# starlingonearth/MASt3R-SLAM-Quality-dualTSDF

Measured on AMD Instinct MI355X. Metric: SLAM frames/sec (infer+match+TSDF+GN) @512x384, higher is better.
Workload: dtype bf16

## Files before the change

include/mslam_hip.h:

```cpp
#ifndef MSLAM_HIP_H
#define MSLAM_HIP_H

#include <stddef.h>
#include <stdint.h>

#ifdef __cplusplus
extern "C" {
#endif

#define MSLAM_OK 0
#define MSLAM_EINVAL (-1)
#define MSLAM_EHIP (-2)
#define MSLAM_ENOMEM (-3)
#define MSLAM_ENODEV (-4)

const char* mslam_last_error(void);
int mslam_abi_version(void);
int mslam_device_check(void);


int mslam_iter_proj(const float* rays_img_with_grad, const float* pts_3d_norm,
                    const float* p_init, float* p_new, uint8_t* converged, int b, int h, int w,
                    int n, int max_iter, float lambda_init, float cost_thresh, void* stream);

// ... 15 lines not shown
int mslam_gauss_newton_rays(float* Twc, const float* Xs, const float* Cs, const int64_t* ii,
                            const int64_t* jj, const int64_t* idx_ii2jj, const uint8_t* valid_match,
                            const float* Q, int num_poses, int num_points, int num_edges,
                            float sigma_ray, float sigma_dist, float C_thresh, float Q_thresh,
                            int max_iter, float delta_thresh, float* dx, void* workspace,
                            size_t workspace_bytes, void* stream);

int mslam_gauss_newton_calib(float* Twc, const float* Xs, const float* Cs, const float* K,
                             const int64_t* ii, const int64_t* jj, const int64_t* idx_ii2jj,
                             const uint8_t* valid_match, const float* Q, int num_poses, int num_points,
                             int num_edges, int height, int width, int pixel_border, float z_eps,
                             float sigma_pixel, float sigma_depth, float C_thresh, float Q_thresh,
                             int max_iter, float delta_thresh, float* dx, void* workspace,
                             size_t workspace_bytes, void* stream);

int mslam_gauss_newton_points(float* Twc, const float* Xs, const float* Cs, const int64_t* ii,
                              const int64_t* jj, const int64_t* idx_ii2jj, const uint8_t* valid_match,
                              const float* Q, int num_poses, int num_points, int num_edges,
                              float sigma_point, float C_thresh, float Q_thresh, int max_iter,
                              float delta_thresh, float* dx, void* workspace, size_t workspace_bytes,
                              void* stream);

int mslam_gn_begin(const int64_t* ii, const int64_t* jj, int num_poses, int num_edges, int num_points,
                   void* workspace, size_t workspace_bytes, void* stream);
int mslam_gn_compact(const float* Xs, const float* Cs, const int64_t* idx_ii2jj, const uint8_t* valid_match,
                     const float* Q, int num_poses, int num_points, int num_edges, int edge_begin,
                     int edge_count, float C_thresh, float Q_thresh, void* workspace, size_t workspace_bytes,
                     void* stream);
int mslam_gn_compact_at(const float* Xs, const float* Cs, const int64_t* idx_ii2jj, const uint8_t* valid_match,
                        const float* Q, int num_poses, int num_points, int num_edges, int edge_begin, int edge_count,
                        int slot_begin, int range_count, float C_thresh, float Q_thresh, void* workspace,
                        size_t workspace_bytes, void* stream);
int mslam_gn_accumulate(int kind, const float* Twc, const float* K, int num_poses, int num_points,
                        int num_edges, int edge_begin, int edge_count, float sigma_a, float sigma_b,
                        int height, int width, int pixel_border, float z_eps, float* Hs, float* gs,
                        void* workspace, size_t workspace_bytes, void* stream);
int mslam_gn_solve_retract(const float* Hs, const float* gs, int num_poses, int num_edges,
                           int num_points, float* Twc, float* dx, float delta_thresh, void* workspace,
                           size_t workspace_bytes, void* stream);
int mslam_gn_status(int* status4, int num_poses, int num_edges, int num_points, void* workspace,
                    size_t workspace_bytes, void* stream);

int mslam_sim3_act(const float* T, const float* X, float* Y, int num_poses, long long pts_per_pose,
                   int broadcast_pose, void* stream);
int mslam_sim3_op(int op, const float* A, const float* B, float* out, int n, int bcast_a, int bcast_b,
                  void* stream);

size_t mslam_tsdf_table_bytes(uint64_t capacity);
int mslam_tsdf_table_init(void* table, size_t table_bytes, uint64_t capacity, void* stream);

size_t mslam_tsdf_integrate_workspace_bytes(int n_points, double voxel_size, double trunc, double step_scale);
int mslam_tsdf_integrate(void* table, uint64_t capacity, const float* points_world, const double* conf,
                         const float* cam_origin, int n_points, double voxel_size, double trunc,
                         double max_weight, double step_scale, int shard_id, int num_shards,
                         void* workspace, size_t workspace_bytes, void* stream);

int mslam_tsdf_rehash(void* old_table, uint64_t old_capacity, void* new_table, uint64_t new_capacity, void* stream);
int mslam_tsdf_header(void* table, uint64_t capacity, uint32_t* out8_host, void* stream);

int mslam_tsdf_dump(void* table, uint64_t capacity, int64_t* keys, double* tsdf, double* weight,
                    uint32_t max_out, void* stream);

int mslam_tsdf_query(void* table, uint64_t capacity, const float* points, int n, double voxel_size,
                     double min_weight, double* value, double* grad, uint8_t* status, void* stream);

int mslam_tsdf_pose_step(void* table, uint64_t capacity, const float* points, const float* conf, int n,
                         float* pose, int points_in_camera_frame, double voxel_size, double min_weight,
                         double lambda, double damping, int update_pose, double* H_out, double* b_out,
                         int* used_out, void* workspace, size_t workspace_bytes, void* stream);

int mslam_tsdf_lookup7(void* table, uint64_t capacity, const float* points, int n, const float* pose,
                       double voxel_size, double* out, void* stream);
int mslam_tsdf_query_lookup(const double* lookup, int n, double voxel_size, double min_weight, double* value,
                            double* grad, uint8_t* status, void* stream);
int mslam_tsdf_pose_step_lookup(const double* lookup, const float* points, const float* conf, int n, float* pose,
                                int points_in_camera_frame, double voxel_size, double min_weight, double lambda,
                                double damping, int update_pose, double* H_out, double* b_out, int* used_out,
                                void* workspace, size_t workspace_bytes, void* stream);

size_t mslam_tsdf_mesh_workspace_bytes(uint64_t capacity);
int mslam_tsdf_mesh_keys(void* table, uint64_t capacity, double min_weight, int64_t* sort_keys, void* stream);
int mslam_tsdf_mesh_count(void* table, uint64_t capacity, double min_weight, double level, const int64_t* sorted_keys,
                          const int64_t* order, int32_t* counts, void* workspace, size_t workspace_bytes, void* stream);
int mslam_tsdf_mesh_emit(void* table, uint64_t capacity, double voxel_size, double min_weight, double level,
                         const int64_t* sorted_keys, const int64_t* order, const int64_t* vbase, const int64_t* fbase,
                         void* workspace, size_t workspace_bytes, float* vertices, float* normals, int32_t* faces,
                         int64_t n_vertices, int64_t n_faces, void* stream);
int mslam_tsdf_load(void* table, uint64_t capacity, const int64_t* keys, const double* tsdf, const double* weight,
                    int n, void* stream);

size_t mslam_tsdf_render_workspace_bytes(uint64_t capacity);
int mslam_tsdf_render_blocks(void* table, uint64_t capacity, double min_weight, void* workspace, size_t workspace_bytes,
                             void* stream);
int mslam_tsdf_render(void* table, uint64_t capacity, const float* rays, int h, int w, const float* pose8,
                      double voxel_size, double min_weight, double level, double near, double far, double step, int skip,
                      const void* workspace, size_t workspace_bytes, float* range, float* normal, uint8_t* hit,
                      void* stream);

size_t mslam_tsdf_color_bytes(uint64_t capacity);
int mslam_tsdf_color_init(void* color, size_t color_bytes, uint64_t capacity, void* stream);
int mslam_tsdf_integrate_color(void* table, uint64_t capacity, void* color, const float* points_world,
                               const double* conf, const float* rgb, const float* cam_origin, int n_points,
                               double voxel_size, double trunc, double step_scale, void* stream);
int mslam_tsdf_color_rehash(void* old_table, uint64_t old_capacity, const void* old_color, void* new_table,
                            uint64_t new_capacity, void* new_color, void* stream);
int mslam_tsdf_color_dump(void* table, uint64_t capacity, const void* color, const int64_t* keys, int n, uint64_t* sums,
                          void* stream);
int mslam_tsdf_color_load(void* table, uint64_t capacity, void* color, const int64_t* keys, const uint64_t* sums, int n,
                          void* stream);
int mslam_tsdf_color_sample(void* table, uint64_t capacity, const void* color, const float* points, int n, int image_w,
                            double voxel_size, double default_r, double default_g, double default_b, float* out_rgb,
                            uint8_t* out_count, void* stream);

int mslam_mast3r_create(void** handle_out, const int* cfg9_host, void* const* weight_ptrs_host,
                        const long long* weight_numels_host, int n_weights, void* stream);
int mslam_mast3r_destroy(void* handle);
size_t mslam_mast3r_workspace_bytes(void* handle, int batch, int H, int W);

int mslam_mast3r_encode(void* handle, const float* img, int batch, int H, int W, float* feat_out,
                        void* workspace, size_t workspace_bytes, void* stream);

int mslam_mast3r_decode(void* handle, const float* feat1, const float* feat2, int batch, int H, int W,
                        float* X1, float* C1, float* D1, float* Q1, float* X2, float* C2, float* D2,
                        float* Q2, float* dec_last1, float* dec_last2, void* workspace,
                        size_t workspace_bytes, void* stream);

size_t mslam_track_workspace_bytes(int n_points);
int mslam_track_pose(int use_calib, float* T_rel, const float* Xf, const float* Xk, const int64_t* idx_f2k,
                     const float* Qk, const uint8_t* valid, int n_points, const float* K, int width,
                     int height, float sigma_a, float sigma_b, float huber, int pixel_border, float z_eps,
                     int first_iter, int max_iters, float rel_error, float delta_norm, void* status_out, void* workspace,
                     size_t workspace_bytes, void* stream);

size_t mslam_track_prepare_workspace_bytes(int n_points);
int mslam_track_prepare(const int64_t* idx_f2k, const uint8_t* valid_match, const float* Qff, const float* Qkf,
                        const float* Cf_sum, float inv_nf, const float* Ck_sum, float inv_nk, float C_conf, float Q_conf,
                        int n_points, const float* T_WCk, const float* T_WCf, float* Qk, float* Ck_avg,
                        uint8_t* valid_opt, uint8_t* valid_kf, float* T_rel, void* workspace, size_t workspace_bytes,
                        void* stream);
int mslam_track_verdict(const void* prepare_workspace, const void* status, int n_points, float* verdict6, void* stream);
int mslam_track_fuse(const float* T_WCk, const float* T_rel, const float* Xkf, const float* Ckf, const float* X_canon,
                     const float* C, int n_points, float* T_WCf, float* X_new, float* C_new, void* stream);

int mslam_gemm_bf16(const void* A, const void* W, const float* bias, const void* residual_f32, void* out,
                    int M, int N, int K, int act, int out_is_bf16, void* stream);
int mslam_gemm_tile_override(int M, int N, int K, int cfg);
int mslam_gemm_profile_begin(int M, int N, int K, int max_samples);
int mslam_gemm_profile_end(double* avg_us, double* min_us, int* samples);
int mslam_conv2d_nhwc_bf16(const void* in, const void* W, const float* bias, const void* residual_bf16,
                           void* out_bf16, int B, int H, int Wd, int Cin, int Cout, int ks, int stride,
                           int relu_in, int act, void* stream);
int mslam_attention_bf16(const void* Q, const void* K, const void* VT, void* O, int batch, int heads,
                         int nq, int nk, void* stream);
int mslam_layernorm_f32(const float* x, const float* w, const float* b, void* out_bf16, float* out_f32,
                        int rows, int D, float eps, void* stream);

size_t mslam_tsdf_local_workspace_bytes(int n_points);
int mslam_tsdf_local_build(const float* X_world, const float* C, const float* origin, const float* xyz_min,
                           const float* xyz_max, int n_points, int nx, int ny, int nz, double voxel_size,
                           double trunc, float min_confidence, float* tsdf, float* weights, void* workspace,
                           size_t workspace_bytes, void* stream);
int mslam_tsdf_local_raycast(const float* tsdf, int nx, int ny, int nz, const float* xyz_min,
                             const float* xyz_max, const float* X_original, const int64_t* sel_pix, int n_sel,
                             int n_samples, float max_displacement, float* surf, uint8_t* hit, void* stream);

int mslam_quality_reduce_grid(const float* x, const float* y, const uint8_t* valid, int h, int w, int ps, int mode,
                              double c_thr, double q_thr, float* out, void* stream);
int mslam_quality_classify(const float* delta_cov, const float* r, const float* u, int n, float thr_zr, float thr_zu,
                           float thr_dc, int64_t* cls, float* pri, void* stream);

int mslam_room_pair(const float* ki, const float* kj, int batch, int h, int w, int n_frames, double fx, double fy,
                    double cx, double cy, double noise, const double* Wm_3x24, const double* phase_24, float* X1,
                    float* C1, float* D1, float* Q1, float* X2, float* C2, float* D2, float* Q2, void* stream);

int mslam_remap_bilinear_u8(const uint8_t* src, int src_h, int src_w, int channels, const float* mapx,
                            const float* mapy, uint8_t* dst, int dst_h, int dst_w, void* stream);

int mslam_gemm_f64(const void* A, int a_is_f32, const void* B, int b_is_f32, int b_transposed, const double* centre,
                   const double* bias, double* out, int M, int N, int K, void* stream);

int mslam_asmk_aggregate(const float* des, const float* centroids, const int64_t* assign, const int64_t* uniq_words,
                         uint32_t* sig_out, int n_des, int m_assign, int dim, int n_uniq, int n_centroids, void* stream);
int mslam_asmk_search(const int32_t* entry_word, const uint32_t* entry_sig, const int32_t* img_start, int n_images,
                      const int32_t* q_words, const uint32_t* q_sig, int n_q, int sig_words, float similarity_threshold,
                      float alpha, double* scores, void* stream);

#ifdef __cplusplus
}
#endif
#endif
```

mast3r-slam-quality-dualtsdf_amd/csrc/attention.hip:

```cpp
#include <stdlib.h>
#include "common.h"
#include "gemm.h"

namespace mslam {

typedef __attribute__((ext_vector_type(8))) __bf16 bf16x8;
typedef __attribute__((ext_vector_type(4))) __bf16 bf16x4;
typedef __attribute__((ext_vector_type(16))) float f32x16;
typedef __attribute__((ext_vector_type(4))) unsigned int u32x4;

constexpr int KV_TILE = 64;
constexpr int AT_STAGE = 16384;
constexpr int OM_ROW = 68;
constexpr unsigned kAtOob = 0x80000000u;

#define MSLAM_LDS_PTR(p) ((__attribute__((address_space(3))) void*)(p))

template <int N>
__device__ __forceinline__ void at_wait_vmcnt() {
  __builtin_amdgcn_s_waitcnt((N & 15) | ((N >> 4) << 14) | 0x0F70);
}

template <int AT_SPLIT>
__global__ __launch_bounds__(128 * AT_SPLIT) void attention_kernel(const bf16* __restrict__ Q, const bf16* __restrict__ K,
                                                        const bf16* __restrict__ VT, bf16* __restrict__ O,
                                                        int heads, int nq, int nk) {
  extern __shared__ __attribute__((aligned(1024))) unsigned char smem[];
  const int t = threadIdx.x, lane = t & 63;
  const int wid = __builtin_amdgcn_readfirstlane(t >> 6);
  const int qg = wid & 1, sp = wid >> 1;
  const int h = lane >> 5, lq = lane & 31;
  const int head = blockIdx.y, b = blockIdx.z;
  const size_t bh = (size_t)b * heads + head;
  const int q_row = blockIdx.x * 64 + qg * 32 + lq;
  const bool q_ok = q_row < nq;

  bf16x8 qf[4];
#pragma unroll
  for (int s = 0; s < 4; s++) {
    const size_t qi = (bh * nq + (q_ok ? q_row : 0)) * 64 + 16 * s + 8 * h;
    qf[s] = __builtin_bit_cast(bf16x8, *reinterpret_cast<const u32x4*>(Q + qi));
  }

  const int ntiles = (nk + KV_TILE - 1) / KV_TILE;
  const int n_iter = (ntiles + AT_SPLIT - 1) / AT_SPLIT;
  const int t_begin = sp * n_iter;
  const int my_n = max(0, min(ntiles, t_begin + n_iter) - t_begin);

  const __amdgpu_buffer_rsrc_t rsK =
      __builtin_amdgcn_make_buffer_rsrc((void*)(K + bh * (size_t)nk * 64), 0, nk * 128, 0x00020000);
  const __amdgpu_buffer_rsrc_t rsV =
      __builtin_amdgcn_make_buffer_rsrc((void*)(VT + bh * 64 * (size_t)nk), 0, nk * 128, 0x00020000);
  const int chunk = (lane & 7) ^ (4 * qg + (lane >> 4));
  unsigned k_off[4], v_off[4];
#pragma unroll
  for (int i = 0; i < 4; i++) {
    const int row = (qg + 2 * i) * 8 + (lane >> 3);
    k_off[i] = (unsigned)(row * 64 + chunk * 8) * 2u;
    v_off[i] = (unsigned)(row * nk + chunk * 8) * 2u;
  }
  auto issue = [&](int stage, int tile) {
    unsigned char* base = smem + (sp * 2 + stage) * AT_STAGE + qg * 1024;
    const int kv0 = tile * KV_TILE;
    const unsigned v_bad = (unsigned)(nk - 1 - (kv0 + chunk * 8)) & kAtOob;
#pragma unroll
    for (int i = 0; i < 4; i++)
      __builtin_amdgcn_raw_ptr_buffer_load_lds(rsK, MSLAM_LDS_PTR(base + i * 2048), 16, k_off[i] + (unsigned)kv0 * 128u, 0, 0, 0);
#pragma unroll
    for (int i = 0; i < 4; i++)
      __builtin_amdgcn_raw_ptr_buffer_load_lds(rsV, MSLAM_LDS_PTR(base + 8192 + i * 2048), 16,
                                               (v_off[i] + (unsigned)kv0 * 2u) | v_bad, 0, 0, 0);
  };

  f32x16 o_acc[2];
#pragma unroll
  for (int dt = 0; dt < 2; dt++)
#pragma unroll
    for (int r = 0; r < 16; r++) o_acc[dt][r] = 0.0f;
  float m_run = -INFINITY, l_run = 0.0f;
  const float kLog2e = 1.4426950408889634f;
  const int kh = h ^ ((lq >> 1) & 7);

  auto compute = [&](int stage, int tile) {
    const unsigned char* sK = smem + (sp * 2 + stage) * AT_STAGE + lq * 128;
    const unsigned char* sV = sK + 8192;
    const int kv0 = tile * KV_TILE;
    f32x16 s_acc[2];
#pragma unroll
    for (int u = 0; u < 2; u++) {
#pragma unroll
      for (int r = 0; r < 16; r++) s_acc[u][r] = 0.0f;
#pragma unroll
      for (int s = 0; s < 4; s++) {
        const bf16x8 kf = *reinterpret_cast<const bf16x8*>(sK + u * 4096 + (((2 * s) ^ kh) * 16));
        s_acc[u] = __builtin_amdgcn_mfma_f32_32x32x16_bf16(kf, qf[s], s_acc[u], 0, 0, 0);
      }
    }
    if (kv0 + KV_TILE > nk) {
#pragma unroll
      for (int u = 0; u < 2; u++)
#pragma unroll
        for (int r = 0; r < 16; r++)
          if (kv0 + 32 * u + (r & 3) + 8 * (r >> 2) + 4 * h >= nk) s_acc[u][r] = -INFINITY;
    }
    float m_tile = -INFINITY;
#pragma unroll
    for (int u = 0; u < 2; u++)
#pragma unroll
      for (int r = 0; r < 16; r++) m_tile = fmaxf(m_tile, s_acc[u][r]);
    m_tile = fmaxf(m_tile, __shfl_xor(m_tile, 32, 64));
    const float m_new = fmaxf(m_run, m_tile);
    const float alpha = __builtin_amdgcn_exp2f((m_run - m_new) * kLog2e);
    const float neg_m = -m_new * kLog2e;
    float l_tile = 0.0f;
#pragma unroll
    for (int u = 0; u < 2; u++)
#pragma unroll
      for (int r = 0; r < 16; r++) {
        const float p = __builtin_amdgcn_exp2f(fmaf(s_acc[u][r], kLog2e, neg_m));
        s_acc[u][r] = p;
        l_tile += p;
      }
    l_tile += __shfl_xor(l_tile, 32, 64);
    l_run = l_run * alpha + l_tile;
    m_run = m_new;
#pragma unroll
    for (int dt = 0; dt < 2; dt++)
#pragma unroll
      for (int r = 0; r < 16; r++) o_acc[dt][r] *= alpha;
#pragma unroll
    for (int u = 0; u < 2; u++) {
#pragma unroll
      for (int s2 = 0; s2 < 2; s2++) {
        bf16x8 pf;
#pragma unroll
        for (int j = 0; j < 8; j++) pf[j] = (bf16)s_acc[u][8 * s2 + j];
        const int c0 = 4 * u + 2 * s2;
#pragma unroll
        for (int dt = 0; dt < 2; dt++) {
          const unsigned char* vrow = sV + dt * 4096 + 8 * h;
          const bf16x4 v0 = *reinterpret_cast<const bf16x4*>(vrow + ((c0 ^ ((lq >> 1) & 7)) * 16));
          const bf16x4 v1 = *reinterpret_cast<const bf16x4*>(vrow + (((c0 + 1) ^ ((lq >> 1) & 7)) * 16));
          bf16x8 vf;
          vf[0] = v0[0]; vf[1] = v0[1]; vf[2] = v0[2]; vf[3] = v0[3];
          vf[4] = v1[0]; vf[5] = v1[1]; vf[6] = v1[2]; vf[7] = v1[3];
          o_acc[dt] = __builtin_amdgcn_mfma_f32_32x32x16_bf16(vf, pf, o_acc[dt], 0, 0, 0);
        }
      }
    }
  };

  if (my_n > 0) issue(0, t_begin);
  if (my_n > 1) issue(1, t_begin + 1);
  for (int i = 0; i < n_iter; i++) {
    if (i == 0 && my_n > 1) at_wait_vmcnt<8>();
    else at_wait_vmcnt<0>();
    __builtin_amdgcn_s_barrier();
    if (i >= 1 && i + 1 < my_n) issue((i + 1) & 1, t_begin + i + 1);
    if (i < my_n) compute(i & 1, t_begin + i);
  }

  __builtin_amdgcn_s_barrier();
  constexpr int NWV = 2 * AT_SPLIT;
  float* Om = reinterpret_cast<float*>(smem);
  float* ml = Om + NWV * 32 * OM_ROW;
  if (h == 0) {
    ml[(wid * 32 + lq) * 2] = m_run;
    ml[(wid * 32 + lq) * 2 + 1] = l_run;
  }
#pragma unroll
  for (int dt = 0; dt < 2; dt++)
#pragma unroll
    for (int gq = 0; gq < 4; gq++)
      *reinterpret_cast<float4*>(Om + (wid * 32 + lq) * OM_ROW + 32 * dt + 8 * gq + 4 * h) =
          make_float4(o_acc[dt][4 * gq], o_acc[dt][4 * gq + 1], o_acc[dt][4 * gq + 2], o_acc[dt][4 * gq + 3]);
  __syncthreads();
  for (int e = t; e < 512; e += 128 * AT_SPLIT) {
    const int q = e >> 3, d0 = (e & 7) * 8;
    const int fq = q >> 5, ql = q & 31;
    float m_s[AT_SPLIT], m_max = -INFINITY;
#pragma unroll
    for (int s = 0; s < AT_SPLIT; s++) {
      m_s[s] = ml[((s * 2 + fq) * 32 + ql) * 2];
      m_max = fmaxf(m_max, m_s[s]);
    }
    float acc8[8] = {0, 0, 0, 0, 0, 0, 0, 0}, l_sum = 0.0f;
#pragma unroll
    for (int s = 0; s < AT_SPLIT; s++) {
      const float w = __builtin_amdgcn_exp2f((m_s[s] - m_max) * kLog2e);
      l_sum = fmaf(w, ml[((s * 2 + fq) * 32 + ql) * 2 + 1], l_sum);
      const float* src = Om + ((s * 2 + fq) * 32 + ql) * OM_ROW + d0;
      const float4 p0 = *reinterpret_cast<const float4*>(src), p1 = *reinterpret_cast<const float4*>(src + 4);
      acc8[0] = fmaf(w, p0.x, acc8[0]); acc8[1] = fmaf(w, p0.y, acc8[1]);
      acc8[2] = fmaf(w, p0.z, acc8[2]); acc8[3] = fmaf(w, p0.w, acc8[3]);
      acc8[4] = fmaf(w, p1.x, acc8[4]); acc8[5] = fmaf(w, p1.y, acc8[5]);
      acc8[6] = fmaf(w, p1.z, acc8[6]); acc8[7] = fmaf(w, p1.w, acc8[7]);
    }
    const int row = blockIdx.x * 64 + q;
    if (row < nq) {
      const float inv = 1.0f / l_sum;
      bf16x8 pk;
#pragma unroll
      for (int k = 0; k < 8; k++) pk[k] = (bf16)(acc8[k] * inv);
      *reinterpret_cast<bf16x8*>(O + ((size_t)b * nq + row) * ((size_t)heads * 64) + (size_t)head * 64 + d0) = pk;
    }
  }
}

template <int AT_SPLIT>
static int launch_attention_split(const bf16* Q, const bf16* K, const bf16* VT, bf16* O, int batch, int heads, int nq,
                                  int nk, hipStream_t stream) {
  constexpr int ring = AT_SPLIT * 2 * AT_STAGE;
  constexpr int merge = (2 * AT_SPLIT * 32 * OM_ROW + 2 * AT_SPLIT * 32 * 2) * (int)sizeof(float);
  constexpr int shmem = ring > merge ? ring : merge;
  static bool attr_set = false;
  if (!attr_set) {
    int rc = check_hip(hipFuncSetAttribute((const void*)attention_kernel<AT_SPLIT>,
                                           hipFuncAttributeMaxDynamicSharedMemorySize, shmem), "attention: attr");
    if (rc) return rc;
    attr_set = true;
  }
  dim3 grid((nq + 63) / 64, heads, batch);
  hipLaunchKernelGGL(attention_kernel<AT_SPLIT>, grid, dim3(128 * AT_SPLIT), shmem, stream, Q, K, VT, O, heads, nq, nk);
  return check_hip(hipGetLastError(), "attention launch");
}

int launch_attention(const bf16* Q, const bf16* K, const bf16* VT, bf16* O, int batch, int heads, int nq, int nk,
                     hipStream_t stream) {
  MSLAM_REQUIRE(nq > 0 && nk > 0 && batch > 0 && heads > 0, "attention: empty problem");
  MSLAM_REQUIRE(nk % 8 == 0, "attention: key count %d must be a multiple of 8", nk);
  MSLAM_REQUIRE((size_t)nk * 128 < (1ull << 31), "attention: key count %d too large", nk);
  static int forced = -2;
  if (forced == -2) {
    const char* e = getenv("MSLAM_ATTN_SPLIT");
    forced = e ? atoi(e) : -1;
  }
  const long blocks = (long)((nq + 63) / 64) * heads * batch;
  const int split = forced > 0 ? forced : (blocks <= 256 ? 4 : 2);
  switch (split) {
    case 4: return launch_attention_split<4>(Q, K, VT, O, batch, heads, nq, nk, stream);
    case 2: return launch_attention_split<2>(Q, K, VT, O, batch, heads, nq, nk, stream);
    default: return launch_attention_split<1>(Q, K, VT, O, batch, heads, nq, nk, stream);
  }
}

}
```

mast3r-slam-quality-dualtsdf_amd/csrc/mast3r.hip:

```cpp
#include <stdlib.h>
#include <vector>
#include "common.h"
#include "gemm.h"

namespace mslam {

int launch_attention(const bf16* Q, const bf16* K, const bf16* VT, bf16* O, int batch, int heads, int nq, int nk,
                     hipStream_t stream);

template <typename TIN>
__global__ __launch_bounds__(256) void layernorm_kernel(const TIN* __restrict__ x, const float* __restrict__ w,
                                                        const float* __restrict__ b, bf16* __restrict__ out_bf,
                                                        float* __restrict__ out_f, int rows, int D, float eps) {
  constexpr int MAXV = 32;
  const int row = blockIdx.x * 4 + (threadIdx.x >> 6);
  const int lane = threadIdx.x & 63;
  if (row >= rows) return;
  const TIN* xr = x + (size_t)row * D;
  float v[MAXV];
  float s = 0.0f;
#pragma unroll
  for (int c = 0; c < MAXV; c++) {
    const int i = lane + 64 * c;
    v[c] = (i < D) ? (float)xr[i] : 0.0f;
    s += v[c];
  }
#pragma unroll
  for (int off = 32; off > 0; off >>= 1) s += __shfl_xor(s, off, 64);
  const float mean = s / (float)D;
  float q = 0.0f;
#pragma unroll
  for (int c = 0; c < MAXV; c++) {
    const float d = (lane + 64 * c < D) ? v[c] - mean : 0.0f;
    q += d * d;
  }
#pragma unroll
  for (int off = 32; off > 0; off >>= 1) q += __shfl_xor(q, off, 64);
  const float rstd = rsqrtf(q / (float)D + eps);
#pragma unroll
  for (int c = 0; c < MAXV; c++) {
    const int i = lane + 64 * c;
    if (i < D) {
      const float y = (v[c] - mean) * rstd * w[i] + b[i];
      if (out_bf) out_bf[(size_t)row * D + i] = (bf16)y;
      if (out_f) out_f[(size_t)row * D + i] = y;
    }
  }
}

typedef __attribute__((ext_vector_type(4))) __bf16 bf16x4;

template <int NV>
__device__ __forceinline__ void ln_load_stats(const float* xrow, int lane, float4 (&v)[NV], float& mean, float& rstd,
                                              float eps) {
  constexpr int D = NV * 256;
  const float4* xr = reinterpret_cast<const float4*>(xrow);
#pragma unroll
  for (int c = 0; c < NV; c++) v[c] = xr[lane + 64 * c];
  float s = 0.0f;
#pragma unroll
  for (int c = 0; c < NV; c++) s += (v[c].x + v[c].y) + (v[c].z + v[c].w);
#pragma unroll
  for (int off = 32; off > 0; off >>= 1) s += __shfl_xor(s, off, 64);
  mean = s / (float)D;
  float q = 0.0f;
#pragma unroll
  for (int c = 0; c < NV; c++) {
    const float dx = v[c].x - mean, dy = v[c].y - mean, dz = v[c].z - mean, dw = v[c].w - mean;
    q += (dx * dx + dy * dy) + (dz * dz + dw * dw);
  }
#pragma unroll
  for (int off = 32; off > 0; off >>= 1) q += __shfl_xor(q, off, 64);
  rstd = rsqrtf(q / (float)D + eps);
}

__device__ __forceinline__ float4 ln_affine(const float4& v, float mean, float rstd, const float4& w, const float4& b) {
  float4 y;
  y.x = (v.x - mean) * rstd * w.x + b.x;
  y.y = (v.y - mean) * rstd * w.y + b.y;
  y.z = (v.z - mean) * rstd * w.z + b.z;
  y.w = (v.w - mean) * rstd * w.w + b.w;
  return y;
}

__device__ __forceinline__ void ln_store_bf16(bf16* out_row, int idx, const float4& y) {
  bf16x4 o;
  o[0] = (bf16)y.x; o[1] = (bf16)y.y; o[2] = (bf16)y.z; o[3] = (bf16)y.w;
  reinterpret_cast<bf16x4*>(out_row)[idx] = o;
}

template <int NV>
__global__ __launch_bounds__(256) void layernorm_vec_kernel(const float* __restrict__ x, const float* __restrict__ w,
                                                            const float* __restrict__ b, bf16* __restrict__ out_bf,
                                                            float* __restrict__ out_f, int rows, float eps) {
  constexpr int D = NV * 256;
  const int row = blockIdx.x * 4 + (threadIdx.x >> 6);
  const int lane = threadIdx.x & 63;
  if (row >= rows) return;
  float4 v[NV], wv[NV], bv[NV];
  float mean, rstd;
#pragma unroll
  for (int c = 0; c < NV; c++) {
    wv[c] = reinterpret_cast<const float4*>(w)[lane + 64 * c];
    bv[c] = reinterpret_cast<const float4*>(b)[lane + 64 * c];
  }
  ln_load_stats<NV>(x + (size_t)row * D, lane, v, mean, rstd, eps);
#pragma unroll
  for (int c = 0; c < NV; c++) {
    const float4 y = ln_affine(v[c], mean, rstd, wv[c], bv[c]);
    if (out_bf) ln_store_bf16(out_bf + (size_t)row * D, lane + 64 * c, y);
    if (out_f) reinterpret_cast<float4*>(out_f + (size_t)row * D)[lane + 64 * c] = y;
  }
}

struct LnSet { const float* w; const float* b; };

template <int NV, bool CROSS>
__global__ __launch_bounds__(256) void layernorm_group_vec_kernel(const float* __restrict__ x, LnSet self0, LnSet self1,
                                                                  LnSet mem0, LnSet mem1, bf16* __restrict__ out_self,
                                                                  bf16* __restrict__ out_mem, int M, float eps) {
  constexpr int D = NV * 256;
  const int row = blockIdx.x * 4 + (threadIdx.x >> 6);
  const int lane = threadIdx.x & 63;
  if (row >= 2 * M) return;
  const int side = row >= M;
  float4 v[NV];
  float mean, rstd;
  ln_load_stats<NV>(x + (size_t)row * D, lane, v, mean, rstd, eps);
#pragma unroll
  for (int k = 0; k < (CROSS ? 2 : 1); k++) {
    const LnSet ps = (k == 0) ? (side ? self1 : self0) : (side ? mem0 : mem1);
    bf16* out = (k == 0) ? out_self + (size_t)row * D : out_mem + (size_t)(side ? row - M : row + M) * D;
#pragma unroll
    for (int c = 0; c < NV; c++) {
      const float4 wv = reinterpret_cast<const float4*>(ps.w)[lane + 64 * c];
      const float4 bv = reinterpret_cast<const float4*>(ps.b)[lane + 64 * c];
      ln_store_bf16(out, lane + 64 * c, ln_affine(v[c], mean, rstd, wv, bv));
    }
  }
}

static void launch_layernorm(const float* x, const float* w, const float* b, bf16* out_bf, float* out_f, int rows, int D,
                             float eps, hipStream_t s) {
  const dim3 grid((rows + 3) / 4), block(256);
  if (D == 1024) hipLaunchKernelGGL(layernorm_vec_kernel<4>, grid, block, 0, s, x, w, b, out_bf, out_f, rows, eps);
  else if (D == 768) hipLaunchKernelGGL(layernorm_vec_kernel<3>, grid, block, 0, s, x, w, b, out_bf, out_f, rows, eps);
  else hipLaunchKernelGGL(layernorm_kernel<float>, grid, block, 0, s, x, w, b, out_bf, out_f, rows, D, eps);
}

__global__ void cast_f32_bf16_kernel(const float* __restrict__ x, bf16* __restrict__ y, size_t n) {
  const size_t i = ((size_t)blockIdx.x * blockDim.x + threadIdx.x) * 4;
  if (i + 3 < n) {
    const float4 v = *reinterpret_cast<const float4*>(x + i);
    bf16x4 o;
    o[0] = (bf16)v.x; o[1] = (bf16)v.y; o[2] = (bf16)v.z; o[3] = (bf16)v.w;
    *reinterpret_cast<bf16x4*>(y + i) = o;
  } else {
    for (size_t k = i; k < n; k++) y[k] = (bf16)x[k];
  }
}

// ... 611 lines not shown
  const int fd = m->fd;
  for (int s = 0; s < 2; s++) {
    Head& h = m->head[s];
    h.a00 = f.lin(dims[0], E, true, "act0.0"); h.a01 = f.lin(dims[0] * 16, dims[0], false, "act0.1");
    h.a01.b = (const float*)f.take(dims[0], "act0.1.bias");
    h.a10 = f.lin(dims[1], D, true, "act1.0"); h.a11 = f.lin(dims[1] * 4, dims[1], false, "act1.1");
    h.a11.b = (const float*)f.take(dims[1], "act1.1.bias");
    h.a20 = f.lin(dims[2], D, true, "act2.0");
    h.a30 = f.lin(dims[3], D, true, "act3.0"); h.a31 = f.lin(dims[3], 9 * dims[3], true, "act3.1");
    for (int k = 0; k < 4; k++) h.rn[k] = f.lin(fd, 9 * dims[k], false, "layer_rn");
    for (int k = 3; k >= 0; k--) {
      Fusion& fu = h.fus[k];
      fu.has_r1 = (k != 3);
      if (fu.has_r1) { fu.r1.c1 = f.lin(fd, 9 * fd, true, "rcu1.conv1"); fu.r1.c2 = f.lin(fd, 9 * fd, true, "rcu1.conv2"); }
      fu.r2.c1 = f.lin(fd, 9 * fd, true, "rcu2.conv1"); fu.r2.c2 = f.lin(fd, 9 * fd, true, "rcu2.conv2");
      fu.out = f.lin(fd, fd, true, "out_conv");
    }
    h.h0 = f.lin(fd / 2, 9 * fd, true, "head.0"); h.h2 = f.lin(fd / 2, 9 * (fd / 2), true, "head.2");
    h.h4w = (const float*)f.take(4 * (fd / 2), "head.4.weight"); h.h4b = (const float*)f.take(4, "head.4.bias");
    const int idim = E + D;
    h.fc1 = f.lin(4 * idim, idim, true, "lf.fc1"); h.fc2 = f.lin((m->desc_dim + 1) * P * P, 4 * idim, true, "lf.fc2");
  }
  if (!f.ok) { delete m; return MSLAM_EINVAL; }
  if (f.pos != n_weights) {
    set_error("mast3r_create: %d weights supplied, %d consumed", n_weights, f.pos);
    delete m;
    return MSLAM_EINVAL;
  }
  m->rope_len = 1024;
  std::vector<float> hc((size_t)m->rope_len * 16), hs((size_t)m->rope_len * 16);
  for (int p = 0; p < m->rope_len; p++)
    for (int i = 0; i < 16; i++) {
      const float inv_freq = 1.0f / powf(100.0f, (float)(2 * i) / 32.0f);
      const float fr = (float)p * inv_freq;
      hc[(size_t)p * 16 + i] = cosf(fr);
      hs[(size_t)p * 16 + i] = sinf(fr);
    }
  int rc = check_hip(hipMalloc(&m->rope_cos, hc.size() * 4 + 16), "rope hipMalloc");
  if (!rc) m->pf_sink = reinterpret_cast<unsigned*>(m->rope_cos + hc.size());
  if (!rc) rc = check_hip(hipMalloc(&m->rope_sin, hs.size() * 4), "rope hipMalloc");
  if (!rc) rc = check_hip(hipMemcpyAsync(m->rope_cos, hc.data(), hc.size() * 4, hipMemcpyHostToDevice, (hipStream_t)stream), "rope copy");
  if (!rc) rc = check_hip(hipMemcpyAsync(m->rope_sin, hs.data(), hs.size() * 4, hipMemcpyHostToDevice, (hipStream_t)stream), "rope copy");
  if (!rc) rc = check_hip(hipStreamSynchronize((hipStream_t)stream), "rope sync");
  if (const char* e = getenv("MSLAM_PREFETCH")) m->prefetch = atoi(e) != 0;
  if (rc) { delete m; return rc; }
  *handle_out = m;
  return MSLAM_OK;
}

extern "C" int mslam_mast3r_destroy(void* handle) {
  Mast3rModel* m = (Mast3rModel*)handle;
  if (!m) return MSLAM_OK;
  if (m->rope_cos) (void)hipFree(m->rope_cos);
  if (m->rope_sin) (void)hipFree(m->rope_sin);
  delete m;
  return MSLAM_OK;
}

static int check_shape(const Mast3rModel* m, int B, int H, int W, const char* who) {
  MSLAM_REQUIRE(m, "%s: null model", who);
  MSLAM_REQUIRE(B >= 1 && H >= m->P && W >= m->P && H % m->P == 0 && W % m->P == 0,
                "%s: image %dx%d must be a positive multiple of the patch size %d", who, H, W, m->P);
  const int N = (H / m->P) * (W / m->P);
  MSLAM_REQUIRE(N % 8 == 0, "%s: token count %d must be a multiple of 8", who, N);
  MSLAM_REQUIRE(m->E <= 2048 && m->Dd <= 2048, "%s: embedding dims above 2048 unsupported", who);
  MSLAM_REQUIRE(H / m->P < m->rope_len && W / m->P < m->rope_len, "%s: token grid exceeds the RoPE table", who);
  return MSLAM_OK;
}

extern "C" size_t mslam_mast3r_workspace_bytes(void* handle, int batch, int H, int W) {
  const Mast3rModel* m = (const Mast3rModel*)handle;
  if (!m || check_shape(m, batch, H, W, "mast3r_workspace_bytes")) return 0;
  Ctx c{m, Arena{nullptr, 0, 0, true}, nullptr};
  encode(c, nullptr, batch, H, W, nullptr);
  c.ar.off = 0;
  HeadOut out[2] = {};
  decode(c, nullptr, nullptr, batch, H, W, out, nullptr, nullptr);
  return c.ar.peak + 4096;
}

extern "C" int mslam_mast3r_encode(void* handle, const float* img, int batch, int H, int W, float* feat_out,
                                   void* workspace, size_t workspace_bytes, void* stream) {
  const Mast3rModel* m = (const Mast3rModel*)handle;
  int rc = check_shape(m, batch, H, W, "mast3r_encode");
  if (rc) return rc;
  MSLAM_REQUIRE(img && feat_out && workspace, "mast3r_encode: null pointer");
  MSLAM_REQUIRE(workspace_bytes >= mslam_mast3r_workspace_bytes(handle, batch, H, W), "mast3r_encode: workspace too small");
  Ctx c{m, Arena{(char*)workspace, 0, workspace_bytes, false}, (hipStream_t)stream};
  encode(c, img, batch, H, W, feat_out);
  MSLAM_REQUIRE(!c.ar.overflow, "mast3r_encode: workspace arena overflow (%zu > %zu)", c.ar.peak, c.ar.cap);
  if (c.rc) return c.rc;
  return check_hip(hipGetLastError(), "mast3r_encode launch");
}

extern "C" int mslam_mast3r_decode(void* handle, const float* feat1, const float* feat2, int batch, int H, int W,
                                   float* X1, float* C1, float* D1, float* Q1, float* X2, float* C2, float* D2,
                                   float* Q2, float* dec_last1, float* dec_last2, void* workspace,
                                   size_t workspace_bytes, void* stream) {
  const Mast3rModel* m = (const Mast3rModel*)handle;
  int rc = check_shape(m, batch, H, W, "mast3r_decode");
  if (rc) return rc;
  MSLAM_REQUIRE(feat1 && feat2 && X1 && C1 && D1 && Q1 && X2 && C2 && D2 && Q2 && workspace, "mast3r_decode: null pointer");
  MSLAM_REQUIRE(workspace_bytes >= mslam_mast3r_workspace_bytes(handle, batch, H, W), "mast3r_decode: workspace too small");
  Ctx c{m, Arena{(char*)workspace, 0, workspace_bytes, false}, (hipStream_t)stream};
  HeadOut out[2] = {{X1, C1, D1, Q1}, {X2, C2, D2, Q2}};
  decode(c, feat1, feat2, batch, H, W, out, dec_last1, dec_last2);
  MSLAM_REQUIRE(!c.ar.overflow, "mast3r_decode: workspace arena overflow (%zu > %zu)", c.ar.peak, c.ar.cap);
  if (c.rc) return c.rc;
  return check_hip(hipGetLastError(), "mast3r_decode launch");
}

extern "C" int mslam_gemm_tile_override(int M, int N, int K, int cfg) {
  MSLAM_REQUIRE(M != 0 && N > 0 && K > 0 && cfg >= 0, "gemm_tile_override: bad arguments");
  return gemm_tile_override(M < 0 ? -M : M, N, K, cfg, M < 0);
}

extern "C" int mslam_gemm_profile_begin(int M, int N, int K, int max_samples) {
  return gemm_profile_begin(M, N, K, max_samples);
}

extern "C" int mslam_gemm_profile_end(double* avg_us, double* min_us, int* samples) {
  return gemm_profile_end(avg_us, min_us, samples);
}

extern "C" int mslam_gemm_bf16(const void* A, const void* Wt, const float* bias, const void* residual_f32, void* out,
                               int M, int N, int K, int act, int out_is_bf16, void* stream) {
  MSLAM_REQUIRE(A && Wt && out, "gemm_bf16: null pointer");
  GemmArgs g = {};
  g.A = (const bf16*)A; g.W = (const bf16*)Wt; g.M = M; g.N = N; g.K = K; g.lda = K; g.bias = bias; g.act = act;
  g.out = out; g.out_kind = out_is_bf16 ? KIND_BF16 : KIND_F32; g.ldc = N; g.ldr1 = N; g.ldr2 = N;
  if (residual_f32) { g.res1 = residual_f32; g.res1_kind = KIND_F32; }
  return launch_gemm(g, (hipStream_t)stream);
}

extern "C" int mslam_conv2d_nhwc_bf16(const void* in, const void* Wt, const float* bias, const void* residual_bf16,
                                      void* out_bf16, int B, int H, int Wd, int Cin, int Cout, int ks, int stride,
                                      int relu_in, int act, void* stream) {
  MSLAM_REQUIRE(in && Wt && out_bf16, "conv2d: null pointer");
  MSLAM_REQUIRE((ks == 1 || ks == 3) && (stride == 1 || stride == 2), "conv2d: unsupported ks/stride");
  Lin l; l.W = (const bf16*)Wt; l.b = bias; l.out = Cout; l.in = ks * ks * Cin;
  GemmArgs g = conv_args((const bf16*)in, B, H, Wd, Cin, l, ks, stride);
  g.out = out_bf16; g.a_relu = relu_in; g.act = act;
  if (residual_bf16) { g.res1 = residual_bf16; g.res1_kind = KIND_BF16; }
  return launch_gemm(g, (hipStream_t)stream);
}

extern "C" int mslam_attention_bf16(const void* Q, const void* K, const void* VT, void* O, int batch, int heads,
                                    int nq, int nk, void* stream) {
  MSLAM_REQUIRE(Q && K && VT && O, "attention: null pointer");
  return launch_attention((const bf16*)Q, (const bf16*)K, (const bf16*)VT, (bf16*)O, batch, heads, nq, nk,
                          (hipStream_t)stream);
}

extern "C" int mslam_layernorm_f32(const float* x, const float* w, const float* b, void* out_bf16, float* out_f32,
                                   int rows, int D, float eps, void* stream) {
  MSLAM_REQUIRE(x && w && b && (out_bf16 || out_f32), "layernorm: null pointer");
  MSLAM_REQUIRE(D <= 2048 && rows > 0, "layernorm: D=%d must be <= 2048", D);
  launch_layernorm(x, w, b, (bf16*)out_bf16, out_f32, rows, D, eps, (hipStream_t)stream);
  MSLAM_LAUNCH_CHECK("layernorm");
  return MSLAM_OK;
}
```

Measured before the change: 166.6.

## Add shared-KV attention kernel with 8 query waves per block for large grids

```diff
diff --git a/include/mslam_hip.h b/include/mslam_hip.h
--- a/include/mslam_hip.h
+++ b/include/mslam_hip.h
@@ -191,6 +191,8 @@
                            int relu_in, int act, void* stream);
 int mslam_attention_bf16(const void* Q, const void* K, const void* VT, void* O, int batch, int heads,
                          int nq, int nk, void* stream);
+int mslam_attention_bf16_variant(const void* Q, const void* K, const void* VT, void* O, int batch, int heads,
+                                 int nq, int nk, int variant, void* stream);
 int mslam_layernorm_f32(const float* x, const float* w, const float* b, void* out_bf16, float* out_f32,
                         int rows, int D, float eps, void* stream);
 
diff --git a/mast3r-slam-quality-dualtsdf_amd/csrc/attention.hip b/mast3r-slam-quality-dualtsdf_amd/csrc/attention.hip
--- a/mast3r-slam-quality-dualtsdf_amd/csrc/attention.hip
+++ b/mast3r-slam-quality-dualtsdf_amd/csrc/attention.hip
@@ -19,6 +19,76 @@
 template <int N>
 __device__ __forceinline__ void at_wait_vmcnt() {
   __builtin_amdgcn_s_waitcnt((N & 15) | ((N >> 4) << 14) | 0x0F70);
+}
+
+__device__ __forceinline__ void at_tile(const unsigned char* sK, int kv0, int nk, const bf16x8 (&qf)[4],
+                                        f32x16 (&o_acc)[2], float& m_run, float& l_run, int lq, int h) {
+  const unsigned char* sV = sK + 8192;
+  const float kLog2e = 1.4426950408889634f;
+  const int kh = h ^ ((lq >> 1) & 7);
+  f32x16 s_acc[2];
+#pragma unroll
+  for (int u = 0; u < 2; u++) {
+#pragma unroll
+    for (int r = 0; r < 16; r++) s_acc[u][r] = 0.0f;
+#pragma unroll
+    for (int s = 0; s < 4; s++) {
+      const bf16x8 kf = *reinterpret_cast<const bf16x8*>(sK + u * 4096 + (((2 * s) ^ kh) * 16));
+      s_acc[u] = __builtin_amdgcn_mfma_f32_32x32x16_bf16(kf, qf[s], s_acc[u], 0, 0, 0);
+    }
+  }
+  if (kv0 + KV_TILE > nk) {
+#pragma unroll
+    for (int u = 0; u < 2; u++)
+#pragma unroll
+      for (int r = 0; r < 16; r++)
+        if (kv0 + 32 * u + (r & 3) + 8 * (r >> 2) + 4 * h >= nk) s_acc[u][r] = -INFINITY;
+  }
+  float m_tile = -INFINITY;
+#pragma unroll
+  for (int u = 0; u < 2; u++)
+#pragma unroll
+    for (int r = 0; r < 16; r++) m_tile = fmaxf(m_tile, s_acc[u][r]);
+  m_tile = fmaxf(m_tile, __shfl_xor(m_tile, 32, 64));
+  const float m_new = fmaxf(m_run, m_tile);
+  const float alpha = __builtin_amdgcn_exp2f((m_run - m_new) * kLog2e);
+  const float neg_m = -m_new * kLog2e;
+  float l_tile = 0.0f;
+#pragma unroll
+  for (int u = 0; u < 2; u++)
+#pragma unroll
+    for (int r = 0; r < 16; r++) {
+      const float p = __builtin_amdgcn_exp2f(fmaf(s_acc[u][r], kLog2e, neg_m));
+      s_acc[u][r] = p;
+      l_tile += p;
+    }
+  l_tile += __shfl_xor(l_tile, 32, 64);
+  l_run = l_run * alpha + l_tile;
+  m_run = m_new;
+#pragma unroll
+  for (int dt = 0; dt < 2; dt++)
+#pragma unroll
+    for (int r = 0; r < 16; r++) o_acc[dt][r] *= alpha;
+#pragma unroll
+  for (int u = 0; u < 2; u++) {
+#pragma unroll
+    for (int s2 = 0; s2 < 2; s2++) {
+      bf16x8 pf;
+#pragma unroll
+      for (int j = 0; j < 8; j++) pf[j] = (bf16)s_acc[u][8 * s2 + j];
+      const int c0 = 4 * u + 2 * s2;
+#pragma unroll
+      for (int dt = 0; dt < 2; dt++) {
+        const unsigned char* vrow = sV + dt * 4096 + 8 * h;
+        const bf16x4 v0 = *reinterpret_cast<const bf16x4*>(vrow + ((c0 ^ ((lq >> 1) & 7)) * 16));
+        const bf16x4 v1 = *reinterpret_cast<const bf16x4*>(vrow + (((c0 + 1) ^ ((lq >> 1) & 7)) * 16));
+        bf16x8 vf;
+        vf[0] = v0[0]; vf[1] = v0[1]; vf[2] = v0[2]; vf[3] = v0[3];
+        vf[4] = v1[0]; vf[5] = v1[1]; vf[6] = v1[2]; vf[7] = v1[3];
+        o_acc[dt] = __builtin_amdgcn_mfma_f32_32x32x16_bf16(vf, pf, o_acc[dt], 0, 0, 0);
+      }
+    }
+  }
 }
 
 template <int AT_SPLIT>
@@ -207,6 +277,102 @@
   }
 }
 
+template <int QW>
+__global__ __launch_bounds__(64 * QW) void attention_shared_kernel(const bf16* __restrict__ Q, const bf16* __restrict__ K,
+                                                                   const bf16* __restrict__ VT, bf16* __restrict__ O,
+                                                                   int heads, int nq, int nk) {
+  extern __shared__ __attribute__((aligned(1024))) unsigned char smem[];
+  constexpr int NP = 8 / QW;
+  const int t = threadIdx.x, lane = t & 63;
+  const int wid = __builtin_amdgcn_readfirstlane(t >> 6);
+  const int h = lane >> 5, lq = lane & 31;
+  const int head = blockIdx.y, b = blockIdx.z;
+  const size_t bh = (size_t)b * heads + head;
+  const int row0 = blockIdx.x * (32 * QW) + wid * 32;
+  const bool q_ok = row0 + lq < nq;
+
+  bf16x8 qf[4];
+#pragma unroll
+  for (int s = 0; s < 4; s++) {
+    const size_t qi = (bh * nq + (q_ok ? row0 + lq : 0)) * 64 + 16 * s + 8 * h;
+    qf[s] = __builtin_bit_cast(bf16x8, *reinterpret_cast<const u32x4*>(Q + qi));
+  }
+  const int ntiles = (nk + KV_TILE - 1) / KV_TILE;
+
+  const __amdgpu_buffer_rsrc_t rsK =
+      __builtin_amdgcn_make_buffer_rsrc((void*)(K + bh * (size_t)nk * 64), 0, nk * 128, 0x00020000);
+  const __amdgpu_buffer_rsrc_t rsV =
+      __builtin_amdgcn_make_buffer_rsrc((void*)(VT + bh * 64 * (size_t)nk), 0, nk * 128, 0x00020000);
+  const int chunk = (lane & 7) ^ (4 * (wid & 1) + (lane >> 4));
+  unsigned k_off[2], v_off[2];
+#pragma unroll
+  for (int i = 0; i < NP; i++) {
+    const int row = (wid + QW * i) * 8 + (lane >> 3);
+    k_off[i] = (unsigned)(row * 64 + chunk * 8) * 2u;
+    v_off[i] = (unsigned)(row * nk + chunk * 8) * 2u;
+  }
+  auto issue = [&](int stage, int tile) {
+    unsigned char* base = smem + stage * AT_STAGE + wid * 1024;
+    const int kv0 = tile * KV_TILE;
+    const unsigned v_bad = (unsigned)(nk - 1 - (kv0 + chunk * 8)) & kAtOob;
+#pragma unroll
+    for (int i = 0; i < NP; i++)
+      __builtin_amdgcn_raw_ptr_buffer_load_lds(rsK, MSLAM_LDS_PTR(base + i * QW * 1024), 16,
+                                               k_off[i] + (unsigned)kv0 * 128u, 0, 0, 0);
+#pragma unroll
+    for (int i = 0; i < NP; i++)
+      __builtin_amdgcn_raw_ptr_buffer_load_lds(rsV, MSLAM_LDS_PTR(base + 8192 + i * QW * 1024), 16,
+                                               (v_off[i] + (unsigned)kv0 * 2u) | v_bad, 0, 0, 0);
+  };
+
+  f32x16 o_acc[2];
+#pragma unroll
+  for (int dt = 0; dt < 2; dt++)
+#pragma unroll
+    for (int r = 0; r < 16; r++) o_acc[dt][r] = 0.0f;
+  float m_run = -INFINITY, l_run = 0.0f;
+
+  issue(0, 0);
+  if (ntiles > 1) issue(1, 1);
+  for (int i = 0; i < ntiles; i++) {
+    if (i == 0 && ntiles > 1) at_wait_vmcnt<2 * NP>();
+    else at_wait_vmcnt<0>();
+    __builtin_amdgcn_s_barrier();
+    if (i >= 1 && i + 1 < ntiles) issue((i + 1) & 1, i + 1);
+    at_tile(smem + (i & 1) * AT_STAGE + lq * 128, i * KV_TILE, nk, qf, o_acc, m_run, l_run, lq, h);
+  }
+
+  __syncthreads();
+  unsigned char* so = smem + wid * 4096;
+  const float inv = 1.0f / l_run;
+#pragma unroll
+  for (int dt = 0; dt < 2; dt++)
+#pragma unroll
+    for (int gq = 0; gq < 4; gq++) {
+      bf16x4 pk;
+#pragma unroll
+      for (int k = 0; k < 4; k++) pk[k] = (bf16)(o_acc[dt][4 * gq + k] * inv);
+      *reinterpret_cast<bf16x4*>(so + lq * 128 + (((4 * dt + gq) ^ (lq & 7)) * 16) + 8 * h) = pk;
+    }
+  __syncthreads();
+#pragma unroll
+  for (int it = 0; it < 4; it++) {
+    const int r = it * 8 + (lane >> 3), c = lane & 7;
+    const u32x4 v = *reinterpret_cast<const u32x4*>(so + r * 128 + ((c ^ (r & 7)) * 16));
+    if (row0 + r < nq)
+      *reinterpret_cast<u32x4*>(O + ((size_t)b * nq + row0 + r) * ((size_t)heads * 64) + (size_t)head * 64 + c * 8) = v;
+  }
+}
+
+template <int QW>
+static int launch_attention_shared(const bf16* Q, const bf16* K, const bf16* VT, bf16* O, int batch, int heads, int nq,
+                                   int nk, hipStream_t stream) {
+  static_assert(QW * 4096 <= 2 * AT_STAGE && 8 / QW <= 2, "the output rows must fit the ring, at most 2 + 2 pieces per wave");
+  dim3 grid((nq + 32 * QW - 1) / (32 * QW), heads, batch);
+  hipLaunchKernelGGL(attention_shared_kernel<QW>, grid, dim3(64 * QW), 2 * AT_STAGE, stream, Q, K, VT, O, heads, nq, nk);
+  return check_hip(hipGetLastError(), "attention launch");
+}
+
 template <int AT_SPLIT>
 static int launch_attention_split(const bf16* Q, const bf16* K, const bf16* VT, bf16* O, int batch, int heads, int nq,
                                   int nk, hipStream_t stream) {
@@ -225,23 +391,34 @@
   return check_hip(hipGetLastError(), "attention launch");
 }
 
-int launch_attention(const bf16* Q, const bf16* K, const bf16* VT, bf16* O, int batch, int heads, int nq, int nk,
-                     hipStream_t stream) {
+int launch_attention_variant(const bf16* Q, const bf16* K, const bf16* VT, bf16* O, int batch, int heads, int nq, int nk,
+                             int variant, hipStream_t stream) {
   MSLAM_REQUIRE(nq > 0 && nk > 0 && batch > 0 && heads > 0, "attention: empty problem");
   MSLAM_REQUIRE(nk % 8 == 0, "attention: key count %d must be a multiple of 8", nk);
   MSLAM_REQUIRE((size_t)nk * 128 < (1ull << 31), "attention: key count %d too large", nk);
+  if (variant == 0) {
+    const long per_row_block = (long)heads * batch;
+    const long blocks = (long)((nq + 63) / 64) * per_row_block;
+    if ((long)((nq + 255) / 256) * per_row_block >= 256) variant = 108;
+    else variant = blocks <= 256 ? 4 : 2;
+  }
+  switch (variant) {
+    case 108: return launch_attention_shared<8>(Q, K, VT, O, batch, heads, nq, nk, stream);
+    case 4: return launch_attention_split<4>(Q, K, VT, O, batch, heads, nq, nk, stream);
+    case 2: return launch_attention_split<2>(Q, K, VT, O, batch, heads, nq, nk, stream);
+    case 1: return launch_attention_split<1>(Q, K, VT, O, batch, heads, nq, nk, stream);
+    default: MSLAM_REQUIRE(false, "attention: unknown variant %d", variant);
+  }
+}
+
+int launch_attention(const bf16* Q, const bf16* K, const bf16* VT, bf16* O, int batch, int heads, int nq, int nk,
+                     hipStream_t stream) {
   static int forced = -2;
   if (forced == -2) {
     const char* e = getenv("MSLAM_ATTN_SPLIT");
     forced = e ? atoi(e) : -1;
   }
-  const long blocks = (long)((nq + 63) / 64) * heads * batch;
-  const int split = forced > 0 ? forced : (blocks <= 256 ? 4 : 2);
-  switch (split) {
-    case 4: return launch_attention_split<4>(Q, K, VT, O, batch, heads, nq, nk, stream);
-    case 2: return launch_attention_split<2>(Q, K, VT, O, batch, heads, nq, nk, stream);
-    default: return launch_attention_split<1>(Q, K, VT, O, batch, heads, nq, nk, stream);
-  }
-}
-
-}
+  return launch_attention_variant(Q, K, VT, O, batch, heads, nq, nk, forced > 0 ? forced : 0, stream);
+}
+
+}
diff --git a/mast3r-slam-quality-dualtsdf_amd/csrc/mast3r.hip b/mast3r-slam-quality-dualtsdf_amd/csrc/mast3r.hip
--- a/mast3r-slam-quality-dualtsdf_amd/csrc/mast3r.hip
+++ b/mast3r-slam-quality-dualtsdf_amd/csrc/mast3r.hip
@@ -7,6 +7,8 @@
 
 int launch_attention(const bf16* Q, const bf16* K, const bf16* VT, bf16* O, int batch, int heads, int nq, int nk,
                      hipStream_t stream);
+int launch_attention_variant(const bf16* Q, const bf16* K, const bf16* VT, bf16* O, int batch, int heads, int nq, int nk,
+                             int variant, hipStream_t stream);
 
 template <typename TIN>
 __global__ __launch_bounds__(256) void layernorm_kernel(const TIN* __restrict__ x, const float* __restrict__ w,
@@ -924,6 +926,13 @@
                           (hipStream_t)stream);
 }
 
+extern "C" int mslam_attention_bf16_variant(const void* Q, const void* K, const void* VT, void* O, int batch, int heads,
+                                            int nq, int nk, int variant, void* stream) {
+  MSLAM_REQUIRE(Q && K && VT && O, "attention: null pointer");
+  return launch_attention_variant((const bf16*)Q, (const bf16*)K, (const bf16*)VT, (bf16*)O, batch, heads, nq, nk,
+                                  variant, (hipStream_t)stream);
+}
+
 extern "C" int mslam_layernorm_f32(const float* x, const float* w, const float* b, void* out_bf16, float* out_f32,
                                    int rows, int D, float eps, void* stream) {
   MSLAM_REQUIRE(x && w && b && (out_bf16 || out_f32), "layernorm: null pointer");
```

After: 160.2. -3.8%, worse.
